# baryshnikova-lab/safepy

Measured on AMD Instinct MI355X. Metric: node-attribute enrichments/sec (nodes x attrs x perms), compute_pvalues permutation test, higher is better.
Workload: dtype u1 (bit-sliced integer counts; f64 outputs)

## Files before the change

### safepy_amd/csrc/attr.hip

```cpp
#include "common.h"

template <typename T>
__device__ __forceinline__ double load_attr(const void *raw, int64_t idx) {
    return static_cast<double>(reinterpret_cast<const T *>(raw)[idx]);
}

template <typename T, int GC>
__global__ __launch_bounds__(256) void k_attr_stats(const void *__restrict__ raw, int64_t n, int64_t m,
                                                    int64_t rs, int64_t cs, unsigned int *__restrict__ row_bits,
                                                    unsigned long long *__restrict__ acc ,
                                                    double *__restrict__ col_sum, unsigned long long *__restrict__ max_abs_bits,
                                                    unsigned int *__restrict__ col_nan, int64_t rows_per_block) {
    extern __shared__ unsigned int s_bits[];
    constexpr int RL = 256 / GC;
    const int cx = GC == 1 ? 0 : (threadIdx.x & (GC - 1));
    const int ry = GC == 1 ? threadIdx.x : (threadIdx.x / GC);
    const int lane = threadIdx.x & 63;
    const int64_t j = static_cast<int64_t>(blockIdx.x) * GC + cx;
    const int64_t n_words = (n + 31) / 32;
    __shared__ double s_sum[256];
    __shared__ double s_max[256];
    __shared__ unsigned int s_nan[256], s_other[256], s_nonint[256];
    const int64_t r_begin = static_cast<int64_t>(blockIdx.y) * rows_per_block;
    const int64_t r_end = r_begin + rows_per_block < n ? r_begin + rows_per_block : n;
// ... 111 lines not shown
            if (s_max[t] > tmx) tmx = s_max[t];
            t_nan += s_nan[t];
            t_other += s_other[t];
            t_nonint += s_nonint[t];
        }
        if (gridDim.y == 1) col_sum[j] = total;
        else atomicAdd(&col_sum[j], total);
        if (t_nan) atomicAdd(&col_nan[j], static_cast<unsigned int>(t_nan));
        if (t_other) atomicAdd(&acc[4 + (j & 63)], t_other);
        if (t_nonint) atomicAdd(&acc[68 + (j & 63)], t_nonint);
        const unsigned long long mine = static_cast<unsigned long long>(__double_as_longlong(tmx));
        if (mine > __builtin_nontemporal_load(max_abs_bits)) atomicMax(max_abs_bits, mine);
    }
}

__global__ __launch_bounds__(256) void k_stats_finish(unsigned long long *__restrict__ acc, const unsigned int *__restrict__ col_nan, int64_t m,
                                                      const unsigned int *__restrict__ bits, int64_t n, uint8_t *__restrict__ bytes,
                                                      unsigned long long *__restrict__ tail) {
    __shared__ unsigned int s_mx[4];
    __shared__ unsigned long long s_fold[2];
    unsigned int mx = 0;
    for (int64_t i = threadIdx.x; i < m; i += 256) mx = col_nan[i] > mx ? col_nan[i] : mx;
    for (int off = 32; off; off >>= 1) {
        const unsigned int o = __shfl_down(mx, off);
        mx = o > mx ? o : mx;
    }
    if ((threadIdx.x & 63) == 0) s_mx[threadIdx.x >> 6] = mx;
    if (threadIdx.x < 64) {
        unsigned long long a = acc[4 + threadIdx.x], b = acc[68 + threadIdx.x];
        for (int off = 32; off; off >>= 1) {
            a += __shfl_down(a, off);
            b += __shfl_down(b, off);
        }
        if (threadIdx.x == 0) s_fold[0] = a, s_fold[1] = b;
    }
    for (int64_t i = threadIdx.x; i < n; i += 256) bytes[i] = (bits[i >> 5] >> (i & 31)) & 1u;
    __syncthreads();
// ... 114 lines not shown
    SAFE_TRY(dev_alloc(&attr->sup_row, total));
    SAFE_HIP_CHECK(hipMemcpyAsync(attr->sup_ptr, attr->h_sup_ptr.data(), (m + 1) * sizeof(int32_t), hipMemcpyHostToDevice,
                                  ctx->stream));
    if (attr->dtype == SAFE_DTYPE_F32)
        hipLaunchKernelGGL(k_fill_support<float>, dim3(ceil_div(m * 64, 256)), dim3(256), 0, ctx->stream, attr->raw, n, m,
                           attr->row_stride, attr->col_stride, attr->sup_ptr, attr->sup_row);
    else
        hipLaunchKernelGGL(k_fill_support<double>, dim3(ceil_div(m * 64, 256)), dim3(256), 0, ctx->stream, attr->raw, n, m,
                           attr->row_stride, attr->col_stride, attr->sup_ptr, attr->sup_row);
    SAFE_HIP_CHECK(hipGetLastError());
    return SAFE_OK;
}

static size_t flags_block_bytes(int64_t n) { return static_cast<size_t>(ceil_div(n, 8)) * 8 + 32; }

int safe_attr_prepare(safe_attr *attr) {
    if (attr->stats_ready) return SAFE_OK;
    safe_ctx *ctx = attr->ctx;
    SAFE_HIP_CHECK(hipSetDevice(ctx->device));
    const int64_t n = attr->n, m = attr->m;
    const size_t flag_bytes = flags_block_bytes(n), tail_off = flag_bytes - 32;
    const int64_t n_words = (n + 31) / 32;
    SAFE_REQUIRE(n_words * sizeof(unsigned int) <= 150 * 1024, "safe_attr_stats: too many rows for the LDS row bitmap");
    void *tmp = nullptr;
    const size_t tmp_bytes = 132 * sizeof(unsigned long long) + static_cast<size_t>(n_words + m) * sizeof(unsigned int);
    SAFE_TRY(ctx_scratch(ctx, SCRATCH_ATTR_STATS, tmp_bytes, &tmp));
    unsigned long long *d_acc = static_cast<unsigned long long *>(tmp);
    unsigned int *d_rowbits = reinterpret_cast<unsigned int *>(d_acc + 132);
    unsigned int *d_colnan = d_rowbits + n_words;
    SAFE_HIP_CHECK(hipMemsetAsync(tmp, 0, tmp_bytes, ctx->stream));
    uint8_t *flags = nullptr;
    SAFE_TRY(ctx_block_alloc(ctx, flag_bytes, reinterpret_cast<void **>(&flags)));
    if (!attr->col_sum) SAFE_TRY(ctx_block_alloc(ctx, static_cast<size_t>(m) * sizeof(double), reinterpret_cast<void **>(&attr->col_sum)));
    const bool f32 = attr->dtype == SAFE_DTYPE_F32;
    const bool c_order = attr->col_stride == 1 && m > 1;
    if (c_order) SAFE_HIP_CHECK(hipMemsetAsync(attr->col_sum, 0, m * sizeof(double), ctx->stream));
#define STATS(T, GC, RPB)                                                                                          \
    do {                                                                                                           \
        if (n_words * sizeof(unsigned int) > 32 * 1024)                                                            \
            SAFE_HIP_CHECK(hipFuncSetAttribute(reinterpret_cast<const void *>(k_attr_stats<T, GC>),                \
                                               hipFuncAttributeMaxDynamicSharedMemorySize,                         \
                                               static_cast<int>(n_words * sizeof(unsigned int))));                 \
        hipLaunchKernelGGL((k_attr_stats<T, GC>), dim3(ceil_div(m, GC), ceil_div(n, RPB)), dim3(256),              \
                           n_words * sizeof(unsigned int), ctx->stream, attr->raw, n, m, attr->row_stride,         \
                           attr->col_stride, d_rowbits, d_acc, attr->col_sum, d_acc + 3, d_colnan,                 \
                           static_cast<int64_t>(RPB));                                                             \
    } while (0)
    if (c_order) {
        const int64_t groups = ceil_div(m, 64);
        const int64_t want_chunks = std::max<int64_t>(1, 2048 / groups);
        const int64_t rpb = std::max<int64_t>(256, ceil_div(ceil_div(n, want_chunks), 64) * 64);
        if (f32) STATS(float, 64, rpb);
        else STATS(double, 64, rpb);
    } else {
        if (f32) STATS(float, 1, n);
        else STATS(double, 1, n);
    }
#undef STATS
    hipLaunchKernelGGL(k_stats_finish, dim3(1), dim3(256), 0, ctx->stream, d_acc, d_colnan, m, d_rowbits, n, flags,
                       reinterpret_cast<unsigned long long *>(flags + tail_off));
    SAFE_HIP_CHECK(hipGetLastError());
    void *pinned = nullptr;
    SAFE_TRY(ctx_pinned(ctx, flag_bytes, &pinned));
    SAFE_HIP_CHECK(hipMemcpyAsync(pinned, flags, flag_bytes, hipMemcpyDeviceToHost, ctx->stream));
    SAFE_HIP_CHECK(safe_stream_sync(ctx->stream));
    const uint8_t *h_flags = static_cast<const uint8_t *>(pinned);
    unsigned long long h_acc[4];
    memcpy(h_acc, h_flags + tail_off, sizeof(h_acc));
    attr->n_other = static_cast<int64_t>(h_acc[0]);
    attr->max_nan_col = static_cast<int64_t>(h_acc[1]);
    attr->n_non_integer = static_cast<int64_t>(h_acc[2]);
    double mx;
    memcpy(&mx, &h_acc[3], sizeof(double));
    attr->max_abs = mx;
    if (!attr->flags_ready) {
        if (attr->row_flags) ctx_block_free(ctx, attr->row_flags, flag_bytes);
        attr->row_flags = flags;
        attr->flags_ready = true;
        int64_t cnt = 0;
        for (int64_t i = 0; i < n; ++i) cnt += h_flags[i] != 0;
        attr->n_rows_with_value = cnt;
        attr->h_row_flags.assign(h_flags, h_flags + n);
    } else {
// ... 387 lines not shown
    SAFE_REQUIRE(attr != nullptr, "safe_attr_nan_to_zero: attr is NULL");
    safe_ctx *ctx = attr->ctx;
    SAFE_HIP_CHECK(hipSetDevice(ctx->device));
    const int64_t count = attr->n * attr->m;
    const unsigned blocks = static_cast<unsigned>(std::min<int64_t>(ceil_div(count, 256), 8192));
    void *raw = const_cast<void *>(attr->raw);
    if (attr->dtype == SAFE_DTYPE_F32)
        hipLaunchKernelGGL(k_nan_to_zero<float>, dim3(blocks), dim3(256), 0, ctx->stream, reinterpret_cast<float *>(raw), count);
    else
        hipLaunchKernelGGL(k_nan_to_zero<double>, dim3(blocks), dim3(256), 0, ctx->stream, reinterpret_cast<double *>(raw), count);
    SAFE_HIP_CHECK(hipGetLastError());
    SAFE_HIP_CHECK(safe_stream_sync(ctx->stream));
    attr->stats_ready = false;
    attr->flags_ready = false;
    attr_free_support(attr);
    return SAFE_OK;
}

int safe_attr_download(safe_attr *attr, void *out_host) {
    SAFE_REQUIRE(attr && out_host, "safe_attr_download: NULL argument");
    safe_ctx *ctx = attr->ctx;
    SAFE_HIP_CHECK(hipSetDevice(ctx->device));
    const size_t bytes = static_cast<size_t>(attr->n) * attr->m * (attr->dtype == SAFE_DTYPE_F32 ? 4 : 8);
    SAFE_HIP_CHECK(hipMemcpyAsync(out_host, attr->raw, bytes, hipMemcpyDeviceToHost, ctx->stream));
    SAFE_HIP_CHECK(safe_stream_sync(ctx->stream));
    return SAFE_OK;
}

int safe_attr_destroy(safe_attr *attr) {
    if (!attr) return SAFE_OK;
    (void)hipSetDevice(attr->ctx->device);
    (void)safe_stream_sync(attr->ctx->stream);
    if (attr->owns_raw && attr->raw_pool_bytes) ctx_block_free(attr->ctx, const_cast<void *>(attr->raw), attr->raw_pool_bytes);
    else if (attr->owns_raw) (void)dev_free(attr->raw);
    ctx_block_free(attr->ctx, attr->row_flags, flags_block_bytes(attr->n));
    ctx_block_free(attr->ctx, attr->col_sum, static_cast<size_t>(attr->m) * sizeof(double));
    attr_free_support(attr);
    delete attr;
    return SAFE_OK;
}

int safe_attr_stats(safe_attr *attr, int64_t *n_other, int64_t *max_nan_col, int64_t *n_rows_with_value,
                    int64_t *n_non_integer) {
    SAFE_REQUIRE(attr != nullptr, "safe_attr_stats: attr is NULL");
    SAFE_TRY(safe_attr_prepare(attr));
    if (n_other) *n_other = attr->n_other;
    if (max_nan_col) *max_nan_col = attr->max_nan_col;
    if (n_rows_with_value) *n_rows_with_value = attr->n_rows_with_value;
    if (n_non_integer) *n_non_integer = attr->n_non_integer;
    return SAFE_OK;
}
// ... 24 lines not shown

int safe_attr_set_row_flags(safe_attr *attr, const uint8_t *flags_host) {
    SAFE_REQUIRE(attr && flags_host, "safe_attr_set_row_flags: NULL argument");
    safe_ctx *ctx = attr->ctx;
    SAFE_HIP_CHECK(hipSetDevice(ctx->device));
    const size_t flag_bytes = flags_block_bytes(attr->n);
    if (!attr->row_flags) SAFE_TRY(ctx_block_alloc(ctx, flag_bytes, reinterpret_cast<void **>(&attr->row_flags)));
    std::vector<uint8_t> tmp(flag_bytes, 0);
    int64_t cnt = 0;
    for (int64_t i = 0; i < attr->n; ++i) {
        tmp[i] = flags_host[i] ? 1 : 0;
        cnt += tmp[i];
    }
    SAFE_HIP_CHECK(hipMemcpyAsync(attr->row_flags, tmp.data(), flag_bytes, hipMemcpyHostToDevice, ctx->stream));
    SAFE_HIP_CHECK(safe_stream_sync(ctx->stream));
    attr->flags_ready = true;
    attr->n_rows_with_value = cnt;
    attr->h_row_flags.assign(tmp.begin(), tmp.begin() + attr->n);
    return SAFE_OK;
}

}
```

### safepy_amd/csrc/common.h

```cpp
#pragma once
#include <hip/hip_runtime.h>

#include <algorithm>
#include <cstdarg>
#include <cmath>
#include <cstdint>
#include <cstdio>
#include <cstdlib>
#include <cstring>
#include <condition_variable>
#include <memory>
#include <mutex>
#include <atomic>
#include <string>
#include <thread>
#include <vector>

#include "safe_hip.h"
#include "bits_plan.h"

#define SAFE_WAVE 64
#define SAFE_PAD_U16 0xFFFFu

void safe_set_error(const char *fmt, ...);
// ... 274 lines not shown
    int32_t *row_ptr = nullptr;
    int32_t *col = nullptr;
    int64_t n_slices = 0;
    int32_t *sell_row = nullptr;
    int32_t *sell_pos = nullptr;
    int64_t *slice_off = nullptr;
    int32_t *slice_width = nullptr;
    int32_t *sell_col = nullptr;
    int64_t sell_entries = 0;
    uint16_t *sell_col2 = nullptr;
    uint16_t *sell_col2b = nullptr;
    std::vector<int32_t> h_slice_width;
    BitsTaskPlan bits_plan;
    void *bits_plan_pinned = nullptr;
    size_t bits_plan_pinned_bytes = 0;
    std::vector<int64_t> h_slice_off;
    std::vector<int32_t> h_row_count;
    double *dist = nullptr;
    int32_t *at_ptr = nullptr;
    int32_t *at_col = nullptr;
    std::vector<double> h_xy;
    bool blocks_ready = false;
    int64_t bs_groups = 0;
    int64_t bs_blocks = 0;
    int64_t bs_pieces = 0;
    int64_t bs_src = 0;
    int32_t *bs_order = nullptr;
    int32_t *bs_rowmap = nullptr;
    int32_t *bs_rowcnt = nullptr;
    int32_t *bs_grpmax = nullptr;
// ... 63 lines not shown
    const void *raw = nullptr;
    bool owns_raw = false;
    size_t raw_pool_bytes = 0;
    uint8_t *row_flags = nullptr;
    std::vector<uint8_t> h_row_flags;
    bool flags_ready = false;
    bool stats_ready = false;
    int64_t n_other = 0, max_nan_col = 0, n_rows_with_value = 0, n_non_integer = 0;
    double *col_sum = nullptr;
    double max_abs = 0.0;
    int32_t *sup_ptr = nullptr;
    int32_t *sup_row = nullptr;
    int64_t n_ones = 0;
    std::vector<int32_t> h_sup_ptr;
    size_t sup_ptr_pool_bytes = 0, sup_row_pool_bytes = 0;
};

struct DrawStream;

struct safe_perms {
    safe_ctx *ctx = nullptr;
    int64_t n = 0;
    int64_t count = 0;
    int64_t k = 0;
    std::vector<int32_t> h_movable;
    DrawStream *stream = nullptr;
    int64_t generated = 0, enqueued = 0;
    std::vector<int64_t> stages;
    std::vector<hipEvent_t> chunk_done;
    std::vector<uint32_t> h_local;
    std::thread drawer;
// ... 98 lines not shown
```

### safepy_amd/csrc/ctx.hip

```cpp
#include "common.h"
#include "ring.h"

#include <atomic>
#include <chrono>
#include <map>
#include <thread>

static thread_local char g_error[1024] = "";

void safe_trace(const char *what) {
    static const bool on = getenv("SAFE_HIP_TRACE") != nullptr;
    if (!on) return;
    static const auto t0 = std::chrono::steady_clock::now();
    fprintf(stderr, "[safe_hip %9.3f ms] %s\n",
            std::chrono::duration<double, std::milli>(std::chrono::steady_clock::now() - t0).count(), what);
}

void safe_warn_diagnostic(const char *name) {
    static std::mutex mu;
    static std::vector<std::string> seen;
    std::lock_guard<std::mutex> lk(mu);
    for (const std::string &n : seen)
        if (n == name) return;
    seen.emplace_back(name);
    fprintf(stderr, "[safe_hip] WARNING: diagnostic switch %s is set: kernels skip work, the results of this process are INVALID\n", name);
}

void safe_set_error(const char *fmt, ...) {
    va_list ap;
    va_start(ap, fmt);
    vsnprintf(g_error, sizeof(g_error), fmt, ap);
    va_end(ap);
}

static std::atomic<int> g_blocking_sync{-1};
std::atomic<long long> g_alloc_calls{0}, g_live_blocks{0};

static bool blocking_sync_on() {
    int v = g_blocking_sync.load(std::memory_order_relaxed);
    if (v < 0) {
// ... 455 lines not shown
```

### safepy_amd/csrc/enrich.hip

```cpp
#include <algorithm>
#include <cmath>
#include <numeric>

#include "common.h"
#include "hyp_math.h"

template <typename T, int BN, int PLANES>
__global__ __launch_bounds__(256) void k_tile_prep(const void *__restrict__ raw, int64_t n, int64_t rs, int64_t cs,
                                                   int64_t col0, int64_t mloc, int64_t n_tiles,
                                                   double *__restrict__ bt) {
    const int64_t idx = static_cast<int64_t>(blockIdx.x) * 256 + threadIdx.x;
    const int64_t total = n_tiles * (n + 1) * BN;
    if (idx >= total) return;
    const int c = static_cast<int>(idx % BN);
    const int64_t row = (idx / BN) % (n + 1);
    const int64_t tile = idx / (static_cast<int64_t>(BN) * (n + 1));
    const int64_t j = tile * BN + c;
    double v = 0.0, v2 = 0.0, nn = 0.0;
    if (row < n && j < mloc) {
        const T x = reinterpret_cast<const T *>(raw)[row * rs + (col0 + j) * cs];
        if (x == x) {
            v = static_cast<double>(x);
            v2 = static_cast<double>(static_cast<T>(x * x));
            nn = 1.0;
// ... 1159 lines not shown
    blk_sum<LV, 2, 1>(ids, lane, nblk, o0, o1);
#pragma unroll
    for (int l = 0; l < BT_LV; ++l) {
        oo0[l] = l < LV ? o0[l < LV ? l : 0] : 0u;
        oo1[l] = l < LV ? o1[l < LV ? l : 0] : 0u;
        obs[l * 64 + lane] = oo0[l];
        obs[(BT_LV + l) * 64 + lane] = oo1[l];
    }
}

__global__ __launch_bounds__(256) void k_bits_observed(int64_t n, const int32_t *__restrict__ sell_row,
                                                       const int64_t *__restrict__ slice_off,
                                                       const int32_t *__restrict__ slice_width,
                                                       const uint16_t *__restrict__ sell_col2b, int64_t n_slices,
                                                       const uint2 *__restrict__ bbits, int64_t mloc,
                                                       uint32_t *__restrict__ obs, double *__restrict__ ns_out) {
    extern __shared__ unsigned int lds[];
    uint2 *T = reinterpret_cast<uint2 *>(lds);
    if ((uint32_t)(uintptr_t)((__attribute__((address_space(3))) unsigned int *)lds) != 0u) __builtin_trap();
    const int wave = __builtin_amdgcn_readfirstlane(threadIdx.x >> 6), lane = threadIdx.x & 63;
    const int64_t wg = blockIdx.x, s = static_cast<int64_t>(blockIdx.y) * 4 + wave;
    load_word_column(T, bbits + wg * (n + 1), n);
    __syncthreads();
    if (s >= n_slices) return;
    const int wdt = __builtin_amdgcn_readfirstlane(slice_width[s]);
    const u32x4 *ids = reinterpret_cast<const u32x4 *>(sell_col2b) + slice_off[s] / 8;
    uint32_t *my_obs = obs + (wg * n_slices + s) * (2 * BT_LV * 64);
    uint32_t oo0[BT_LV], oo1[BT_LV];
    if (wdt <= 8) observed_wave<4>(ids, lane, wdt >> 3, my_obs, oo0, oo1);
    else if (wdt <= 56) observed_wave<6>(ids, lane, wdt >> 3, my_obs, oo0, oo1);
    else if (wdt <= 248) observed_wave<8>(ids, lane, wdt >> 3, my_obs, oo0, oo1);
    else if (wdt <= 504) observed_wave<9>(ids, lane, wdt >> 3, my_obs, oo0, oo1);
    else observed_wave<BT_LV>(ids, lane, wdt >> 3, my_obs, oo0, oo1);
    if (ns_out) {
        const int32_t row = sell_row[s * 64 + lane];
        uint16_t *tile = reinterpret_cast<uint16_t *>(lds + 2 * ((n + 2) & ~int64_t(1)) + 4) + wave * (64 * 66);
// ... 343 lines not shown
    const int64_t n = attr->n;
    const bool f32 = attr->dtype == SAFE_DTYPE_F32;
    if (attr->col_stride == 1 && attr->row_stride != 1) {
        const dim3 grid(n_wg, ceil_div(n + 1, 4)), block(256);
        if (f32) hipLaunchKernelGGL(k_bits_prep_rowmajor<float>, grid, block, 0, ctx->stream, attr->raw, n, attr->row_stride,
                                    attr->col_stride, col0, mloc, n_wg, d_bits);
        else hipLaunchKernelGGL(k_bits_prep_rowmajor<double>, grid, block, 0, ctx->stream, attr->raw, n, attr->row_stride,
                                attr->col_stride, col0, mloc, n_wg, d_bits);
    } else {
        const dim3 grid(ceil_div(n_wg * (n + 1), 256)), block(256);
        if (f32) hipLaunchKernelGGL(k_bits_prep<float>, grid, block, 0, ctx->stream, attr->raw, n, attr->row_stride,
                                    attr->col_stride, col0, mloc, n_wg, d_bits);
        else hipLaunchKernelGGL(k_bits_prep<double>, grid, block, 0, ctx->stream, attr->raw, n, attr->row_stride,
                                attr->col_stride, col0, mloc, n_wg, d_bits);
    }
}


template <bool TABLE>
__global__ __launch_bounds__(64) void k_counts_bits(const int32_t *__restrict__ sell_row,
                                                    const int64_t *__restrict__ slice_off,
                                                    const int32_t *__restrict__ slice_width,
                                                    const int32_t *__restrict__ sell_col, int64_t n,
                                                    const uint2 *__restrict__ bbits, int64_t mloc,
                                                    double *__restrict__ out, HypLookup hl) {
    const int64_t s = blockIdx.x, wg = blockIdx.y;
    const int lane = threadIdx.x;
    const int32_t row = sell_row[s * 64 + lane];
    const int32_t *cols = sell_col + slice_off[s] + lane;
    const int wdt = slice_width[s];
// ... 582 lines not shown
                        tail.n_major, tail.n_chunks, tail.wpc);
    const std::vector<int4> &recs = bits_plan_records(plan, form);
    const size_t bytes = recs.size() * sizeof(int4);
    if (nbr->bits_plan_pinned_bytes < bytes) {
        SAFE_HIP_CHECK(safe_stream_sync(ctx->stream));
        if (nbr->bits_plan_pinned) SAFE_HIP_CHECK(hipHostFree(nbr->bits_plan_pinned));
        nbr->bits_plan_pinned = nullptr;
        nbr->bits_plan_pinned_bytes = 0;
        g_alloc_calls.fetch_add(1, std::memory_order_relaxed);
        SAFE_HIP_CHECK(hipHostMalloc(&nbr->bits_plan_pinned, bytes + 4096, hipHostMallocDefault));
        nbr->bits_plan_pinned_bytes = bytes + 4096;
    } else {
        SAFE_HIP_CHECK(safe_stream_sync(ctx->stream));
    }
    memcpy(nbr->bits_plan_pinned, recs.data(), bytes);
    plan.key = plan_key;
    return SAFE_OK;
}

constexpr int BITS_NS = 2;

struct BitsBuffers {
    uint2 *d_bits = nullptr;
    int4 *d_tasks = nullptr;
    unsigned int *d_queue = nullptr, *d_gl = nullptr;
    int64_t n_pad = 0, entries_pad = 0;
    uint16_t *d_ids[BITS_NS] = {nullptr, nullptr};
    uint16_t *d_ids_tail = nullptr;
    uint32_t *d_obs = nullptr;
};
static int bits_call_buffers(safe_ctx *ctx, const safe_nbr *nbr, const BitsForm &form, const BitsTail &tail, int64_t mloc, int64_t span,
                             int64_t tail_span, BitsBuffers *b) {
    const size_t n_task = bits_plan_records(nbr->bits_plan, form).size();
    const int64_t n_launch = tail.n_major + tail.n_chunks;
    void *ws = nullptr;
    SAFE_TRY(ctx_scratch(ctx, SCRATCH_TASKS, n_task * sizeof(int4) + (8 * n_launch + 4) * sizeof(unsigned int), &ws));
    b->d_tasks = static_cast<int4 *>(ws);
    b->d_queue = reinterpret_cast<unsigned int *>(b->d_tasks + n_task);
    b->n_pad = nbr->n_slices * 64;
    SAFE_TRY(ctx_scratch(ctx, SCRATCH_COUNTERS, static_cast<size_t>(b->n_pad) * mloc * sizeof(unsigned int), reinterpret_cast<void **>(&b->d_gl)));
    SAFE_HIP_CHECK(hipMemcpyAsync(b->d_tasks, nbr->bits_plan_pinned, n_task * sizeof(int4), hipMemcpyHostToDevice, ctx->stream));
    SAFE_HIP_CHECK(hipMemsetAsync(b->d_queue, 0, 8 * n_launch * sizeof(unsigned int), ctx->stream));
    SAFE_HIP_CHECK(hipMemsetAsync(b->d_gl, 0, static_cast<size_t>(b->n_pad) * mloc * sizeof(unsigned int), ctx->stream));
    safe_trace("launch_bits: buffers ready");
    b->entries_pad = (nbr->sell_entries + 1024 + 255) / 256 * 256;
    for (int s = 0; s < BITS_NS; ++s)
        SAFE_TRY(ctx_scratch(ctx, scratch_pair(SCRATCH_STREAM_A, s), static_cast<size_t>(span) * b->entries_pad * sizeof(uint16_t), reinterpret_cast<void **>(&b->d_ids[s])));
    if (tail.n_chunks)
        SAFE_TRY(ctx_scratch(ctx, SCRATCH_BITS_TAIL_IDS, static_cast<size_t>(tail_span) * b->entries_pad * sizeof(uint16_t), reinterpret_cast<void **>(&b->d_ids_tail)));
    return SAFE_OK;
}

static int bits_observe(safe_ctx *ctx, const safe_nbr *nbr, const BitsForm &form, int64_t mloc, double *ns_out, BitsBuffers *b) {
    const int64_t n_wg = ceil_div(mloc, 64);
    SAFE_TRY(ctx_scratch(ctx, SCRATCH_BITS_OBSERVED, static_cast<size_t>(n_wg) * nbr->n_slices * 2 * BT_LV * 64 * sizeof(uint32_t),
                         reinterpret_cast<void **>(&b->d_obs)));
    const size_t lds_obs = form.lds_bytes + (ns_out ? 4 * 64 * 66 * sizeof(uint16_t) : 0);
    SAFE_HIP_CHECK(hipFuncSetAttribute(reinterpret_cast<const void *>(k_bits_observed), hipFuncAttributeMaxDynamicSharedMemorySize,
                                       static_cast<int>(lds_obs)));
    hipLaunchKernelGGL(k_bits_observed, dim3(n_wg, ceil_div(nbr->n_slices, 4)), dim3(256), lds_obs, ctx->stream, nbr->n, nbr->sell_row,
                       nbr->slice_off, nbr->slice_width, nbr->sell_col2b, nbr->n_slices, b->d_bits, mloc, b->d_obs, ns_out);
    SAFE_HIP_CHECK(hipGetLastError());
    return SAFE_OK;
}

static int bits_tail_lists(safe_ctx *ctx, const safe_nbr *nbr, safe_perms *perms, const std::vector<int64_t> &starts, const BitsTail &tail,
                           const BitsBuffers &b, hipEvent_t *plain) {
    hipStream_t tail_ps = ctx->more_streams[1], kstreams[BITS_NS] = {ctx->stream, ctx->side_stream};
    const int64_t n_stage = static_cast<int64_t>(starts.size()) - 1, entries_pad = b.entries_pad;
    SAFE_HIP_CHECK(hipStreamWaitEvent(tail_ps, plain[0], 0));
    for (int64_t t = tail.n_major; t < n_stage; ++t) {
        SAFE_TRY(perms_wait(perms, starts[t + 1], tail_ps));
        hipLaunchKernelGGL(k_permute_cols, dim3(ceil_div(entries_pad, 4096), starts[t + 1] - starts[t]), dim3(256),
                           static_cast<size_t>(perms->stride16) * sizeof(uint16_t), tail_ps, perms->table16, perms->stride16,
                           nbr->sell_col2b, nbr->sell_entries, entries_pad, starts[t], starts[t + 1] - starts[t],
                           static_cast<uint32_t>(8 * nbr->n), b.d_ids_tail + (starts[t] - tail.p_split) * entries_pad, 3);
// ... 53 lines not shown
                            (void *)&n_pad};
        void *pre_args[] = {(void *)&n, (void *)&ids_c, (void *)&entries_pad, (void *)&nbr->sell_row, (void *)&nbr->slice_off,
                            (void *)&nbr->slice_width, (void *)&nbr->sell_col2, (void *)&nbr->n_slices, (void *)&b.d_bits, (void *)&n_tasks,
                            (void *)&d_tasks, (void *)&p_base, (void *)&p_limit, (void *)&queue_c, (void *)&mloc, (void *)&b.d_gl,
                            (void *)&n_pad, (void *)&ns_out};
        SAFE_HIP_CHECK(hipLaunchKernel(kfn, dim3(grid), dim3(form.block), blk ? blk_args : pre_args, form.lds_bytes, ks));
        if (in_tail) chunk_final(c, ks);
        SAFE_HIP_CHECK(hipGetLastError());
        SAFE_HIP_CHECK(hipEventRecord(fr.ev[2 * c + 1], ks));
    }
    return SAFE_OK;
}

static int launch_bits(safe_ctx *ctx, safe_nbr *nbr, safe_attr *attr, safe_perms *perms, int64_t col0, int64_t col1,
                       const PermOut &out) {
    const int64_t n = nbr->n, mloc = col1 - col0, n_wg = ceil_div(mloc, 64), P = perms->count;
    const BitsForm form = bits_form(n, nbr->max_count, nbr->sell_col2 != nullptr, 160 * 1024);
    SAFE_REQUIRE(form.kind != BITS_NONE, "launch_bits: no bit-sliced form for %lld nodes with neighborhoods of up to %lld members",
                 static_cast<long long>(n), static_cast<long long>(nbr->max_count));
    safe_trace("launch_bits: enter");
    BitsBuffers b;
    SAFE_TRY(ctx_scratch(ctx, SCRATCH_OPERANDS, static_cast<size_t>(n_wg) * (n + 1) * sizeof(uint2), reinterpret_cast<void **>(&b.d_bits)));
    launch_bits_prep(ctx, attr, col0, mloc, n_wg, b.d_bits);
    safe_trace("launch_bits: prep launched");
    const BitsSwitches sw = bits_switches(ctx);
    int64_t span = 1;
    const std::vector<int64_t> starts = perm_launch_starts(perms, &span, 1, sw.tail_frac > 0.0);
    ctx->xc_made = 0;
    const BitsTail tail = bits_tail_split(ctx->xc_want, ctx->xc_cols, safe_ctx::XC_MAX, form.kind == BITS_BLK, starts, P, mloc, sw.tail_frac);
    const int64_t n_tail = tail.n_chunks, tail_span = P - tail.p_split;
    const int64_t n_launch = tail.n_major + n_tail;
    const int per_cu = static_cast<int>(std::max<size_t>(1, std::min<size_t>(8, (160 * 1024) / bits_lds_bytes(n, perms->stride16))));
    SAFE_TRY(bits_task_plan(ctx, nbr, form, tail, starts, static_cast<int64_t>(ctx->num_cu) * per_cu, mloc));
    safe_trace("launch_bits: tasks built");
    SAFE_TRY(bits_call_buffers(ctx, nbr, form, tail, mloc, span, tail_span, &b));
    const void *kfn = bits_form_kernel(form, sw.dbg);
    if (!kfn) return SAFE_E_INVALID;
    SAFE_HIP_CHECK(hipFuncSetAttribute(kfn, hipFuncAttributeMaxDynamicSharedMemorySize, static_cast<int>(form.lds_bytes)));
// ... 18 lines not shown
        safe_trace("launch_bits: column chunks enqueued");
        if (ctx->xc_callback) ctx->xc_callback(ctx->xc_user);
    }
    SAFE_TRY(span_frame_join(ctx, fr));
    SAFE_TRY(enrich_finalize_counts(ctx, b.d_gl, b.n_pad, nbr->sell_row, mloc, P, out, nullptr));
    SAFE_HIP_CHECK(hipGetLastError());
    safe_trace("launch_bits: all enqueued");
    SAFE_TRY(span_frame_close(ctx, fr));
    safe_trace("launch_bits: synced");
    if (sw.dbg & 128) blk_trace_dump(static_cast<int>(n_launch));
    return SAFE_OK;
}

static int launch_counts_bits(safe_ctx *ctx, safe_nbr *nbr, safe_attr *attr, int64_t col0, int64_t col1, double *out_dev) {
    const int64_t n = nbr->n, mloc = col1 - col0, n_wg = ceil_div(mloc, 64);
    uint2 *d_bits = nullptr;
    SAFE_TRY(ctx_scratch(ctx, SCRATCH_OPERANDS, static_cast<size_t>(n_wg) * (n + 1) * sizeof(uint2), reinterpret_cast<void **>(&d_bits)));
    launch_bits_prep(ctx, attr, col0, mloc, n_wg, d_bits);
    SAFE_HIP_CHECK(hipEventRecord(ctx->k0, ctx->stream));
    hipLaunchKernelGGL(k_counts_bits<false>, dim3(nbr->n_slices, n_wg), dim3(64), 0, ctx->stream, nbr->sell_row, nbr->slice_off,
                       nbr->slice_width, nbr->sell_col, n, d_bits, mloc, out_dev, HypLookup{});
    SAFE_HIP_CHECK(hipGetLastError());
    SAFE_HIP_CHECK(hipEventRecord(ctx->k1, ctx->stream));
    ctx->last_kernel.name = "k_counts_bits";
    return SAFE_OK;
}

static size_t ldsf64_bytes(int64_t n, int64_t stride16) {
    return (8 * static_cast<size_t>(n + 1) + static_cast<size_t>(stride16) + 4) * sizeof(unsigned int);
}

static int launch_lds_f64(safe_ctx *ctx, safe_nbr *nbr, safe_attr *attr, safe_perms *perms, int64_t col0, int64_t col1,
                          bool z, const PermOut &out_in) {
// ... 136 lines not shown
    hl.nes = nes_dev;
    hl.nes_binary = nb_dev;
    hl.enriched = d_enr;
    if (split) {
        int rc = mfma_counts_split_emit(ctx, nbr, split, hl);
        if (rc == SAFE_OK && enriched_f64) {
            hipLaunchKernelGGL(k_u32_to_f64, dim3(ceil_div(mloc, 256)), dim3(256), 0, ctx->stream, d_enr, enriched_f64, mloc);
            if (hipGetLastError() != hipSuccess) rc = SAFE_E_HIP;
        }
        (void)safe_stream_sync(hs);
        (void)hipEventDestroy(ids_done);
        SAFE_TRY(rc);
    } else if (use_mfma) {
        SAFE_TRY(launch_mfma_counts(ctx, nbr, attr, col0, col1, hl));
    } else {
        uint2 *d_bits = nullptr;
        SAFE_TRY(ctx_scratch(ctx, SCRATCH_OPERANDS, static_cast<size_t>(n_wg) * (n + 1) * sizeof(uint2), reinterpret_cast<void **>(&d_bits)));
        launch_bits_prep(ctx, attr, col0, mloc, n_wg, d_bits);
        SAFE_HIP_CHECK(hipEventRecord(ctx->k0, ctx->stream));
        hipLaunchKernelGGL(k_counts_bits<true>, dim3(nbr->n_slices, n_wg), dim3(64), 0, ctx->stream, nbr->sell_row, nbr->slice_off,
                           nbr->slice_width, nbr->sell_col, n, d_bits, mloc, static_cast<double *>(nullptr), hl);
        SAFE_HIP_CHECK(hipGetLastError());
        SAFE_HIP_CHECK(hipEventRecord(ctx->k1, ctx->stream));
        ctx->last_kernel.name = "k_counts_bits<hypergeom>";
    }
    if (split && enriched_f64 && enriched_done) *enriched_done = true;
    SAFE_HIP_CHECK(safe_stream_sync(ctx->stream));
    *fused = true;
    return SAFE_OK;
}

__global__ __launch_bounds__(256) void k_counts_to_outputs(const double *__restrict__ counts_neg, const double *__restrict__ counts_pos,
                                                           const double *__restrict__ ns, int64_t total, int64_t m, int64_t n_perm,
// ... 553 lines not shown
```

### safepy_amd/csrc/nbr.hip

```cpp
#include <algorithm>
#include <cmath>
#include <numeric>

#include "common.h"

static double squared_threshold(double nr) {
    if (!(nr > 0.0)) return 0.0;
    if (std::isinf(nr)) return nr;
    double c = nr * nr;
    if (std::isinf(c)) return c;
    while (c > 0.0 && std::sqrt(c) >= nr) c = std::nextafter(c, 0.0);
    while (std::sqrt(c) < nr) c = std::nextafter(c, INFINITY);
    return c;
}

__global__ __launch_bounds__(256) void k_euclid_bits(const double *__restrict__ xy, int64_t n, double thr_sq,
                                                     uint64_t *__restrict__ bits, int64_t words) {
    __shared__ double sx[64], sy[64];
    const int64_t w = blockIdx.x;
    const int64_t i = static_cast<int64_t>(blockIdx.y) * 256 + threadIdx.x;
    const int64_t j0 = w * 64;
    if (threadIdx.x < 64) {
        const int64_t j = j0 + threadIdx.x;
        sx[threadIdx.x] = j < n ? xy[2 * j] : 0.0;
// ... 600 lines not shown
    }
    SAFE_REQUIRE(src.n >= 2 || n_ranks == 0, "%s: rank %lld is outside [0, 0): one node has no pair", who, (long long)ranks[0]);
    *keys = pre;
    return SAFE_OK;
}

static void nbr_free(safe_nbr *nbr) {
    if (!nbr) return;
    for (const void *q : {(const void *)nbr->bits, (const void *)nbr->row_ptr, (const void *)nbr->col, (const void *)nbr->sell_row,
                          (const void *)nbr->sell_pos, (const void *)nbr->slice_off, (const void *)nbr->slice_width,
                          (const void *)nbr->sell_col, (const void *)nbr->sell_col2, (const void *)nbr->sell_col2b,
                          (const void *)nbr->dist, (const void *)nbr->at_ptr, (const void *)nbr->at_col})
        (void)dev_free(q);
    nbr_free_blocks(nbr);
    if (nbr->bits_plan_pinned) (void)hipHostFree(nbr->bits_plan_pinned);
    delete nbr;
}

using NbrPtr = std::unique_ptr<safe_nbr, void (*)(safe_nbr *)>;

static int nbr_new(safe_ctx *ctx, int64_t n, NbrPtr *out) {
    SAFE_REQUIRE(n >= 1 && n < (1ll << 31) - 64, "neighborhood size n=%lld out of range", (long long)n);
    NbrPtr nbr(new safe_nbr(), nbr_free);
    nbr->ctx = ctx;
    nbr->n = n;
    nbr->words = ceil_div(n, 64);
    SAFE_TRY(dev_alloc(&nbr->bits, static_cast<size_t>(n) * nbr->words));
    *out = std::move(nbr);
    return SAFE_OK;
}
// ... 550 lines not shown
```

Measured before the change: 6892 billion.

## Build attribute bit planes during stats sweep and fold buffer clears into observe kernel

Adds a binary-attribute sweep kernel that computes column statistics and packs the 64-column bit planes in one pass over the raw matrix. Later bit-sliced count launches reuse these cached planes instead of rerunning the bits-prep kernel per call. The task plan is kept resident on the device, and the counter and queue zeroing moves into the observed-counts kernel, removing per-call H2D copies and memsets. If the attribute is not strictly binary, the sweep falls back to the old stats pass, costing an extra pass and some memory for the planes.

After: 6988 billion (median of 6 runs). 1.01x the previous value.

```diff
diff --git a/safepy_amd/csrc/attr.hip b/safepy_amd/csrc/attr.hip
--- a/safepy_amd/csrc/attr.hip
+++ b/safepy_amd/csrc/attr.hip
@@ -1,4 +1,5 @@
 #include "common.h"
+#include "attr_plan.h"
 
 template <typename T>
 __device__ __forceinline__ double load_attr(const void *raw, int64_t idx) {
@@ -149,13 +150,92 @@
     }
 }
 
+template <typename T>
+__global__ __launch_bounds__(256) void k_attr_sweep(const T *__restrict__ raw, int64_t n, int64_t m, int64_t cs, int64_t rows_per_block,
+                                                    unsigned int *__restrict__ row_bits, unsigned long long *__restrict__ acc,
+                                                    unsigned int *__restrict__ col_nan, unsigned int *__restrict__ col_one,
+                                                    uint2 *__restrict__ bbits) {
+    __shared__ unsigned int s_nan[4][64], s_one[4][64], s_other[4];
+    const int wave = threadIdx.x >> 6, lane = threadIdx.x & 63;
+    const int64_t wg = blockIdx.x, j0 = wg * 64;
+    const int n_cols = static_cast<int>(m - j0 < 64 ? m - j0 : 64);
+    const int64_t r_begin = static_cast<int64_t>(blockIdx.y) * rows_per_block;
+    const int64_t r_end = r_begin + rows_per_block < n ? r_begin + rows_per_block : n;
+    const T *base = raw + j0 * cs;
+    uint2 *planes = bbits + wg * (n + 1);
+    unsigned int c_nan = 0, c_one = 0, c_other = 0;
+    for (int64_t r0 = r_begin + wave * 64; r0 < r_end; r0 += 256) {
+        const int64_t r = r0 + lane;
+        const bool inb = r < n;
+        const T *p = base + (inb ? r : r0);
+        uint32_t w0 = 0, w1 = 0;
+        bool has = false;
+        auto take = [&](int a, T v) {
+            const bool nan = v != v, one = v == static_cast<T>(1), zero = v == static_cast<T>(0);
+            const bool is_nan = inb && nan, is_one = inb && one;
+            const unsigned int k_nan = __popcll(__ballot(is_nan)), k_one = __popcll(__ballot(is_one));
+            c_nan += lane == a ? k_nan : 0u;
+            c_one += lane == a ? k_one : 0u;
+            c_other += (inb && !nan && !one && !zero) ? 1u : 0u;
+            has = has || (inb && !nan);
+            if (a < 32) w0 |= (is_one ? 1u : 0u) << (a & 31);
+            else w1 |= (is_one ? 1u : 0u) << (a & 31);
+        };
+        if (n_cols == 64) {
+#pragma unroll
+            for (int a0 = 0; a0 < 64; a0 += 16) {
+                T x[16];
+#pragma unroll
+                for (int u = 0; u < 16; ++u) x[u] = p[(a0 + u) * cs];
+#pragma unroll
+                for (int u = 0; u < 16; ++u) take(a0 + u, x[u]);
+            }
+        } else {
+            for (int a = 0; a < n_cols; ++a) take(a, p[a * cs]);
+        }
+        if (inb) planes[r] = make_uint2(w0, w1);
+        const unsigned long long bal = __ballot(has);
+        if (lane == 0 && bal) {
+            const unsigned int lo = static_cast<unsigned int>(bal), hi = static_cast<unsigned int>(bal >> 32);
+            if (lo & ~row_bits[r0 >> 5]) atomicOr(&row_bits[r0 >> 5], lo);
+            if (hi && (hi & ~row_bits[(r0 >> 5) + 1])) atomicOr(&row_bits[(r0 >> 5) + 1], hi);
+        }
+    }
+    for (int off = 32; off; off >>= 1) c_other += __shfl_down(c_other, off);
+    s_nan[wave][lane] = c_nan;
+    s_one[wave][lane] = c_one;
+    if (lane == 0) s_other[wave] = c_other;
+    __syncthreads();
+    if (threadIdx.x < 64) {
+        const unsigned int t_nan = s_nan[0][lane] + s_nan[1][lane] + s_nan[2][lane] + s_nan[3][lane];
+        const unsigned int t_one = s_one[0][lane] + s_one[1][lane] + s_one[2][lane] + s_one[3][lane];
+        if (lane < n_cols) {
+            if (t_nan) atomicAdd(&col_nan[j0 + lane], t_nan);
+            if (t_one) atomicAdd(&col_one[j0 + lane], t_one);
+        }
+        const bool any_one = __ballot(lane < n_cols && t_one != 0) != 0ull;
+        if (lane == 0) {
+            const unsigned long long t_other = static_cast<unsigned long long>(s_other[0]) + s_other[1] + s_other[2] + s_other[3];
+            if (t_other) atomicAdd(&acc[4 + (wg & 63)], t_other);
+            const unsigned long long one_bits = static_cast<unsigned long long>(__double_as_longlong(1.0));
+            if (any_one && one_bits > __builtin_nontemporal_load(&acc[3])) atomicMax(&acc[3], one_bits);
+            if (blockIdx.y == 0) planes[n] = make_uint2(0u, 0u);
+        }
+    }
+}
+
 __global__ __launch_bounds__(256) void k_stats_finish(unsigned long long *__restrict__ acc, const unsigned int *__restrict__ col_nan, int64_t m,
                                                       const unsigned int *__restrict__ bits, int64_t n, uint8_t *__restrict__ bytes,
-                                                      unsigned long long *__restrict__ tail) {
+                                                      unsigned long long *__restrict__ tail, const unsigned int *__restrict__ col_one,
+                                                      double *__restrict__ col_sum) {
     __shared__ unsigned int s_mx[4];
     __shared__ unsigned long long s_fold[2];
     unsigned int mx = 0;
-    for (int64_t i = threadIdx.x; i < m; i += 256) mx = col_nan[i] > mx ? col_nan[i] : mx;
+    for (int64_t i = threadIdx.x; i < m; i += 256) {
+        const unsigned int c = col_nan[i];
+        if (col_one) col_sum[i] = static_cast<double>(col_one[i]);
+        mx = c > mx ? c : mx;
+    }
     for (int off = 32; off; off >>= 1) {
         const unsigned int o = __shfl_down(mx, off);
         mx = o > mx ? o : mx;
@@ -300,25 +380,47 @@
 
 static size_t flags_block_bytes(int64_t n) { return static_cast<size_t>(ceil_div(n, 8)) * 8 + 32; }
 
-int safe_attr_prepare(safe_attr *attr) {
-    if (attr->stats_ready) return SAFE_OK;
+void attr_drop_planes(safe_attr *attr) {
+    ctx_block_free(attr->ctx, attr->planes, attr->planes_bytes);
+    attr->planes = nullptr;
+    attr->planes_bytes = 0;
+}
+
+const uint2 *attr_bit_planes(const safe_attr *attr, int64_t col0, int64_t col1) {
+    if (!attr->planes || !binary_head_on() || !planes_serve_block(col0, col1, attr->m)) return nullptr;
+    return attr->planes + (col0 / 64) * (attr->n + 1);
+}
+
+static int stats_pass(safe_attr *attr, bool sweep, uint8_t *flags, void *pinned) {
     safe_ctx *ctx = attr->ctx;
-    SAFE_HIP_CHECK(hipSetDevice(ctx->device));
     const int64_t n = attr->n, m = attr->m;
     const size_t flag_bytes = flags_block_bytes(n), tail_off = flag_bytes - 32;
     const int64_t n_words = (n + 31) / 32;
-    SAFE_REQUIRE(n_words * sizeof(unsigned int) <= 150 * 1024, "safe_attr_stats: too many rows for the LDS row bitmap");
     void *tmp = nullptr;
-    const size_t tmp_bytes = 132 * sizeof(unsigned long long) + static_cast<size_t>(n_words + m) * sizeof(unsigned int);
+    const size_t tmp_bytes = 132 * sizeof(unsigned long long) + static_cast<size_t>(n_words + 2 * m) * sizeof(unsigned int);
     SAFE_TRY(ctx_scratch(ctx, SCRATCH_ATTR_STATS, tmp_bytes, &tmp));
     unsigned long long *d_acc = static_cast<unsigned long long *>(tmp);
     unsigned int *d_rowbits = reinterpret_cast<unsigned int *>(d_acc + 132);
-    unsigned int *d_colnan = d_rowbits + n_words;
+    unsigned int *d_colnan = d_rowbits + n_words, *d_colone = d_colnan + m;
     SAFE_HIP_CHECK(hipMemsetAsync(tmp, 0, tmp_bytes, ctx->stream));
-    uint8_t *flags = nullptr;
-    SAFE_TRY(ctx_block_alloc(ctx, flag_bytes, reinterpret_cast<void **>(&flags)));
-    if (!attr->col_sum) SAFE_TRY(ctx_block_alloc(ctx, static_cast<size_t>(m) * sizeof(double), reinterpret_cast<void **>(&attr->col_sum)));
     const bool f32 = attr->dtype == SAFE_DTYPE_F32;
+    if (sweep) {
+        const int64_t n_wg = ceil_div(m, 64), rpb = sweep_rows_per_block(n, n_wg);
+        const dim3 grid(static_cast<unsigned int>(n_wg), static_cast<unsigned int>(ceil_div(n, rpb)));
+        if (f32)
+            hipLaunchKernelGGL(k_attr_sweep<float>, grid, dim3(256), 0, ctx->stream, static_cast<const float *>(attr->raw), n, m,
+                               attr->col_stride, rpb, d_rowbits, d_acc, d_colnan, d_colone, attr->planes);
+        else
+            hipLaunchKernelGGL(k_attr_sweep<double>, grid, dim3(256), 0, ctx->stream, static_cast<const double *>(attr->raw), n, m,
+                               attr->col_stride, rpb, d_rowbits, d_acc, d_colnan, d_colone, attr->planes);
+        hipLaunchKernelGGL(k_stats_finish, dim3(1), dim3(256), 0, ctx->stream, d_acc, d_colnan, m, d_rowbits, n, flags,
+                           reinterpret_cast<unsigned long long *>(flags + tail_off), d_colone, attr->col_sum);
+        SAFE_HIP_CHECK(hipGetLastError());
+        SAFE_HIP_CHECK(hipMemcpyAsync(pinned, flags, flag_bytes, hipMemcpyDeviceToHost, ctx->stream));
+        SAFE_HIP_CHECK(safe_stream_sync(ctx->stream));
+        return SAFE_OK;
+    }
+    SAFE_REQUIRE(n_words * sizeof(unsigned int) <= 150 * 1024, "safe_attr_stats: too many rows for the LDS row bitmap");
     const bool c_order = attr->col_stride == 1 && m > 1;
     if (c_order) SAFE_HIP_CHECK(hipMemsetAsync(attr->col_sum, 0, m * sizeof(double), ctx->stream));
 #define STATS(T, GC, RPB)                                                                                          \
@@ -344,15 +446,41 @@
     }
 #undef STATS
     hipLaunchKernelGGL(k_stats_finish, dim3(1), dim3(256), 0, ctx->stream, d_acc, d_colnan, m, d_rowbits, n, flags,
-                       reinterpret_cast<unsigned long long *>(flags + tail_off));
+                       reinterpret_cast<unsigned long long *>(flags + tail_off), static_cast<const unsigned int *>(nullptr),
+                       static_cast<double *>(nullptr));
     SAFE_HIP_CHECK(hipGetLastError());
+    SAFE_HIP_CHECK(hipMemcpyAsync(pinned, flags, flag_bytes, hipMemcpyDeviceToHost, ctx->stream));
+    SAFE_HIP_CHECK(safe_stream_sync(ctx->stream));
+    return SAFE_OK;
+}
+
+int safe_attr_prepare(safe_attr *attr) {
+    if (attr->stats_ready) return SAFE_OK;
+    safe_ctx *ctx = attr->ctx;
+    SAFE_HIP_CHECK(hipSetDevice(ctx->device));
+    const int64_t n = attr->n, m = attr->m;
+    const size_t flag_bytes = flags_block_bytes(n), tail_off = flag_bytes - 32;
+    SAFE_REQUIRE(static_cast<size_t>((n + 31) / 32) * sizeof(unsigned int) <= 150 * 1024, "safe_attr_stats: too many rows for the LDS row bitmap");
+    uint8_t *flags = nullptr;
+    SAFE_TRY(ctx_block_alloc(ctx, flag_bytes, reinterpret_cast<void **>(&flags)));
+    if (!attr->col_sum) SAFE_TRY(ctx_block_alloc(ctx, static_cast<size_t>(m) * sizeof(double), reinterpret_cast<void **>(&attr->col_sum)));
     void *pinned = nullptr;
     SAFE_TRY(ctx_pinned(ctx, flag_bytes, &pinned));
-    SAFE_HIP_CHECK(hipMemcpyAsync(pinned, flags, flag_bytes, hipMemcpyDeviceToHost, ctx->stream));
-    SAFE_HIP_CHECK(safe_stream_sync(ctx->stream));
     const uint8_t *h_flags = static_cast<const uint8_t *>(pinned);
     unsigned long long h_acc[4];
+    bool sweep = binary_head_on() && attr->row_stride == 1 && (attr->col_stride == n || m == 1);
+    if (sweep && !attr->planes) {
+        const size_t bytes = static_cast<size_t>(ceil_div(m, 64)) * (n + 1) * sizeof(uint2);
+        SAFE_TRY(ctx_block_alloc(ctx, bytes, reinterpret_cast<void **>(&attr->planes)));
+        attr->planes_bytes = bytes;
+    }
+    SAFE_TRY(stats_pass(attr, sweep, flags, pinned));
     memcpy(h_acc, h_flags + tail_off, sizeof(h_acc));
+    if (sweep && h_acc[0] != 0) {
+        attr_drop_planes(attr);
+        SAFE_TRY(stats_pass(attr, false, flags, pinned));
+        memcpy(h_acc, h_flags + tail_off, sizeof(h_acc));
+    }
     attr->n_other = static_cast<int64_t>(h_acc[0]);
     attr->max_nan_col = static_cast<int64_t>(h_acc[1]);
     attr->n_non_integer = static_cast<int64_t>(h_acc[2]);
@@ -770,6 +898,7 @@
     attr->stats_ready = false;
     attr->flags_ready = false;
     attr_free_support(attr);
+    attr_drop_planes(attr);
     return SAFE_OK;
 }
 
@@ -791,6 +920,7 @@
     else if (attr->owns_raw) (void)dev_free(attr->raw);
     ctx_block_free(attr->ctx, attr->row_flags, flags_block_bytes(attr->n));
     ctx_block_free(attr->ctx, attr->col_sum, static_cast<size_t>(attr->m) * sizeof(double));
+    attr_drop_planes(attr);
     attr_free_support(attr);
     delete attr;
     return SAFE_OK;
@@ -845,6 +975,7 @@
     }
     SAFE_HIP_CHECK(hipMemcpyAsync(attr->row_flags, tmp.data(), flag_bytes, hipMemcpyHostToDevice, ctx->stream));
     SAFE_HIP_CHECK(safe_stream_sync(ctx->stream));
+    attr_drop_planes(attr);
     attr->flags_ready = true;
     attr->n_rows_with_value = cnt;
     attr->h_row_flags.assign(tmp.begin(), tmp.begin() + attr->n);
diff --git a/safepy_amd/csrc/attr_plan.h b/safepy_amd/csrc/attr_plan.h
--- /dev/null
+++ b/safepy_amd/csrc/attr_plan.h
@@ -0,0 +1,14 @@
+#pragma once
+#include <cstdint>
+
+static inline int64_t sweep_rows_per_block(int64_t n, int64_t n_wg) {
+    const int64_t chunks = n_wg >= 1024 ? 1 : 1024 / (n_wg < 1 ? 1 : n_wg);
+    const int64_t rows = (n + chunks - 1) / chunks;
+    const int64_t rounded = (rows + 128) / 256 * 256;
+    return rounded < 256 ? 256 : rounded;
+}
+
+static inline bool planes_serve_block(int64_t col0, int64_t col1, int64_t m) {
+    if (col0 < 0 || col1 <= col0 || col1 > m) return false;
+    return col0 % 64 == 0 && (col1 == m || col1 % 64 == 0);
+}
diff --git a/safepy_amd/csrc/common.h b/safepy_amd/csrc/common.h
--- a/safepy_amd/csrc/common.h
+++ b/safepy_amd/csrc/common.h
@@ -312,6 +312,8 @@
     BitsTaskPlan bits_plan;
     void *bits_plan_pinned = nullptr;
     size_t bits_plan_pinned_bytes = 0;
+    int4 *bits_plan_dev = nullptr;
+    size_t bits_plan_dev_bytes = 0;
     std::vector<int64_t> h_slice_off;
     std::vector<int32_t> h_row_count;
     double *dist = nullptr;
@@ -405,7 +407,12 @@
     int64_t n_ones = 0;
     std::vector<int32_t> h_sup_ptr;
     size_t sup_ptr_pool_bytes = 0, sup_row_pool_bytes = 0;
-};
+    uint2 *planes = nullptr;
+    size_t planes_bytes = 0;
+};
+const uint2 *attr_bit_planes(const safe_attr *attr, int64_t col0, int64_t col1);
+void attr_drop_planes(safe_attr *attr);
+bool binary_head_on();
 
 struct DrawStream;
 
diff --git a/safepy_amd/csrc/ctx.hip b/safepy_amd/csrc/ctx.hip
--- a/safepy_amd/csrc/ctx.hip
+++ b/safepy_amd/csrc/ctx.hip
@@ -24,6 +24,11 @@
         if (n == name) return;
     seen.emplace_back(name);
     fprintf(stderr, "[safe_hip] WARNING: diagnostic switch %s is set: kernels skip work, the results of this process are INVALID\n", name);
+}
+
+bool binary_head_on() {
+    const char *e = getenv("SAFE_HIP_BINARY_HEAD");
+    return !(e && !strcmp(e, "0"));
 }
 
 void safe_set_error(const char *fmt, ...) {
diff --git a/safepy_amd/csrc/enrich.hip b/safepy_amd/csrc/enrich.hip
--- a/safepy_amd/csrc/enrich.hip
+++ b/safepy_amd/csrc/enrich.hip
@@ -1197,12 +1197,21 @@
                                                        const int32_t *__restrict__ slice_width,
                                                        const uint16_t *__restrict__ sell_col2b, int64_t n_slices,
                                                        const uint2 *__restrict__ bbits, int64_t mloc,
-                                                       uint32_t *__restrict__ obs, double *__restrict__ ns_out) {
+                                                       uint32_t *__restrict__ obs, double *__restrict__ ns_out,
+                                                       unsigned int *__restrict__ gl_counts, int64_t n_pad,
+                                                       unsigned int *__restrict__ queue, int n_queue) {
     extern __shared__ unsigned int lds[];
     uint2 *T = reinterpret_cast<uint2 *>(lds);
     if ((uint32_t)(uintptr_t)((__attribute__((address_space(3))) unsigned int *)lds) != 0u) __builtin_trap();
     const int wave = __builtin_amdgcn_readfirstlane(threadIdx.x >> 6), lane = threadIdx.x & 63;
     const int64_t wg = blockIdx.x, s = static_cast<int64_t>(blockIdx.y) * 4 + wave;
+    if (gl_counts && s < n_slices) {
+        const int n_valid = static_cast<int>(mloc - wg * 64 < 64 ? mloc - wg * 64 : 64);
+        unsigned int *z = gl_counts + wg * 64 * n_pad + s * 64 + 4 * (lane & 15);
+        for (int a = lane >> 4; a < n_valid; a += 4) *reinterpret_cast<uint4 *>(z + static_cast<int64_t>(a) * n_pad) = make_uint4(0u, 0u, 0u, 0u);
+    }
+    if (queue && blockIdx.x == 0 && blockIdx.y == 0)
+        for (int i = threadIdx.x; i < n_queue; i += 256) queue[i] = 0u;
     load_word_column(T, bbits + wg * (n + 1), n);
     __syncthreads();
     if (s >= n_slices) return;
@@ -1576,6 +1585,19 @@
         else hipLaunchKernelGGL(k_bits_prep<double>, grid, block, 0, ctx->stream, attr->raw, n, attr->row_stride,
                                 attr->col_stride, col0, mloc, n_wg, d_bits);
     }
+}
+
+static int bits_operand(safe_ctx *ctx, const safe_attr *attr, int64_t col0, int64_t col1, const uint2 **out) {
+    if (const uint2 *planes = attr_bit_planes(attr, col0, col1)) {
+        *out = planes;
+        return SAFE_OK;
+    }
+    const int64_t mloc = col1 - col0, n_wg = ceil_div(mloc, 64);
+    uint2 *d_bits = nullptr;
+    SAFE_TRY(ctx_scratch(ctx, SCRATCH_OPERANDS, static_cast<size_t>(n_wg) * (attr->n + 1) * sizeof(uint2), reinterpret_cast<void **>(&d_bits)));
+    launch_bits_prep(ctx, attr, col0, mloc, n_wg, d_bits);
+    *out = d_bits;
+    return SAFE_OK;
 }
 
 
@@ -2188,6 +2210,15 @@
         SAFE_HIP_CHECK(safe_stream_sync(ctx->stream));
     }
     memcpy(nbr->bits_plan_pinned, recs.data(), bytes);
+    if (nbr->bits_plan_dev_bytes < bytes) {
+        SAFE_HIP_CHECK(dev_free(nbr->bits_plan_dev));
+        nbr->bits_plan_dev = nullptr;
+        nbr->bits_plan_dev_bytes = 0;
+        SAFE_TRY(dev_alloc_bytes(reinterpret_cast<void **>(&nbr->bits_plan_dev), bytes + 4096));
+        nbr->bits_plan_dev_bytes = bytes + 4096;
+    }
+    SAFE_HIP_CHECK(hipMemcpyAsync(nbr->bits_plan_dev, nbr->bits_plan_pinned, bytes, hipMemcpyHostToDevice, ctx->stream));
+    SAFE_HIP_CHECK(safe_stream_sync(ctx->stream));
     plan.key = plan_key;
     return SAFE_OK;
 }
@@ -2195,13 +2226,15 @@
 constexpr int BITS_NS = 2;
 
 struct BitsBuffers {
-    uint2 *d_bits = nullptr;
+    const uint2 *d_bits = nullptr;
     int4 *d_tasks = nullptr;
     unsigned int *d_queue = nullptr, *d_gl = nullptr;
     int64_t n_pad = 0, entries_pad = 0;
     uint16_t *d_ids[BITS_NS] = {nullptr, nullptr};
     uint16_t *d_ids_tail = nullptr;
     uint32_t *d_obs = nullptr;
+    bool cleared_by_observe = false;
+    int n_queue = 0;
 };
 static int bits_call_buffers(safe_ctx *ctx, const safe_nbr *nbr, const BitsForm &form, const BitsTail &tail, int64_t mloc, int64_t span,
                              int64_t tail_span, BitsBuffers *b) {
@@ -2213,9 +2246,15 @@
     b->d_queue = reinterpret_cast<unsigned int *>(b->d_tasks + n_task);
     b->n_pad = nbr->n_slices * 64;
     SAFE_TRY(ctx_scratch(ctx, SCRATCH_COUNTERS, static_cast<size_t>(b->n_pad) * mloc * sizeof(unsigned int), reinterpret_cast<void **>(&b->d_gl)));
-    SAFE_HIP_CHECK(hipMemcpyAsync(b->d_tasks, nbr->bits_plan_pinned, n_task * sizeof(int4), hipMemcpyHostToDevice, ctx->stream));
-    SAFE_HIP_CHECK(hipMemsetAsync(b->d_queue, 0, 8 * n_launch * sizeof(unsigned int), ctx->stream));
-    SAFE_HIP_CHECK(hipMemsetAsync(b->d_gl, 0, static_cast<size_t>(b->n_pad) * mloc * sizeof(unsigned int), ctx->stream));
+    const bool head = binary_head_on();
+    b->cleared_by_observe = head && form.kind == BITS_BLK;
+    if (head) b->d_tasks = nbr->bits_plan_dev;
+    else SAFE_HIP_CHECK(hipMemcpyAsync(b->d_tasks, nbr->bits_plan_pinned, n_task * sizeof(int4), hipMemcpyHostToDevice, ctx->stream));
+    if (!b->cleared_by_observe) {
+        SAFE_HIP_CHECK(hipMemsetAsync(b->d_queue, 0, 8 * n_launch * sizeof(unsigned int), ctx->stream));
+        SAFE_HIP_CHECK(hipMemsetAsync(b->d_gl, 0, static_cast<size_t>(b->n_pad) * mloc * sizeof(unsigned int), ctx->stream));
+    }
+    b->n_queue = static_cast<int>(8 * n_launch);
     safe_trace("launch_bits: buffers ready");
     b->entries_pad = (nbr->sell_entries + 1024 + 255) / 256 * 256;
     for (int s = 0; s < BITS_NS; ++s)
@@ -2233,7 +2272,9 @@
     SAFE_HIP_CHECK(hipFuncSetAttribute(reinterpret_cast<const void *>(k_bits_observed), hipFuncAttributeMaxDynamicSharedMemorySize,
                                        static_cast<int>(lds_obs)));
     hipLaunchKernelGGL(k_bits_observed, dim3(n_wg, ceil_div(nbr->n_slices, 4)), dim3(256), lds_obs, ctx->stream, nbr->n, nbr->sell_row,
-                       nbr->slice_off, nbr->slice_width, nbr->sell_col2b, nbr->n_slices, b->d_bits, mloc, b->d_obs, ns_out);
+                       nbr->slice_off, nbr->slice_width, nbr->sell_col2b, nbr->n_slices, b->d_bits, mloc, b->d_obs, ns_out,
+                       b->cleared_by_observe ? b->d_gl : static_cast<unsigned int *>(nullptr), b->n_pad,
+                       b->cleared_by_observe ? b->d_queue : static_cast<unsigned int *>(nullptr), b->n_queue);
     SAFE_HIP_CHECK(hipGetLastError());
     return SAFE_OK;
 }
@@ -2317,14 +2358,13 @@
 
 static int launch_bits(safe_ctx *ctx, safe_nbr *nbr, safe_attr *attr, safe_perms *perms, int64_t col0, int64_t col1,
                        const PermOut &out) {
-    const int64_t n = nbr->n, mloc = col1 - col0, n_wg = ceil_div(mloc, 64), P = perms->count;
+    const int64_t n = nbr->n, mloc = col1 - col0, P = perms->count;
     const BitsForm form = bits_form(n, nbr->max_count, nbr->sell_col2 != nullptr, 160 * 1024);
     SAFE_REQUIRE(form.kind != BITS_NONE, "launch_bits: no bit-sliced form for %lld nodes with neighborhoods of up to %lld members",
                  static_cast<long long>(n), static_cast<long long>(nbr->max_count));
     safe_trace("launch_bits: enter");
     BitsBuffers b;
-    SAFE_TRY(ctx_scratch(ctx, SCRATCH_OPERANDS, static_cast<size_t>(n_wg) * (n + 1) * sizeof(uint2), reinterpret_cast<void **>(&b.d_bits)));
-    launch_bits_prep(ctx, attr, col0, mloc, n_wg, b.d_bits);
+    SAFE_TRY(bits_operand(ctx, attr, col0, col1, &b.d_bits));
     safe_trace("launch_bits: prep launched");
     const BitsSwitches sw = bits_switches(ctx);
     int64_t span = 1;
@@ -2373,9 +2413,8 @@
 
 static int launch_counts_bits(safe_ctx *ctx, safe_nbr *nbr, safe_attr *attr, int64_t col0, int64_t col1, double *out_dev) {
     const int64_t n = nbr->n, mloc = col1 - col0, n_wg = ceil_div(mloc, 64);
-    uint2 *d_bits = nullptr;
-    SAFE_TRY(ctx_scratch(ctx, SCRATCH_OPERANDS, static_cast<size_t>(n_wg) * (n + 1) * sizeof(uint2), reinterpret_cast<void **>(&d_bits)));
-    launch_bits_prep(ctx, attr, col0, mloc, n_wg, d_bits);
+    const uint2 *d_bits = nullptr;
+    SAFE_TRY(bits_operand(ctx, attr, col0, col1, &d_bits));
     SAFE_HIP_CHECK(hipEventRecord(ctx->k0, ctx->stream));
     hipLaunchKernelGGL(k_counts_bits<false>, dim3(nbr->n_slices, n_wg), dim3(64), 0, ctx->stream, nbr->sell_row, nbr->slice_off,
                        nbr->slice_width, nbr->sell_col, n, d_bits, mloc, out_dev, HypLookup{});
@@ -2542,9 +2581,8 @@
     } else if (use_mfma) {
         SAFE_TRY(launch_mfma_counts(ctx, nbr, attr, col0, col1, hl));
     } else {
-        uint2 *d_bits = nullptr;
-        SAFE_TRY(ctx_scratch(ctx, SCRATCH_OPERANDS, static_cast<size_t>(n_wg) * (n + 1) * sizeof(uint2), reinterpret_cast<void **>(&d_bits)));
-        launch_bits_prep(ctx, attr, col0, mloc, n_wg, d_bits);
+        const uint2 *d_bits = nullptr;
+        SAFE_TRY(bits_operand(ctx, attr, col0, col1, &d_bits));
         SAFE_HIP_CHECK(hipEventRecord(ctx->k0, ctx->stream));
         hipLaunchKernelGGL(k_counts_bits<true>, dim3(nbr->n_slices, n_wg), dim3(64), 0, ctx->stream, nbr->sell_row, nbr->slice_off,
                            nbr->slice_width, nbr->sell_col, n, d_bits, mloc, static_cast<double *>(nullptr), hl);
diff --git a/safepy_amd/csrc/nbr.hip b/safepy_amd/csrc/nbr.hip
--- a/safepy_amd/csrc/nbr.hip
+++ b/safepy_amd/csrc/nbr.hip
@@ -638,6 +638,7 @@
         (void)dev_free(q);
     nbr_free_blocks(nbr);
     if (nbr->bits_plan_pinned) (void)hipHostFree(nbr->bits_plan_pinned);
+    (void)dev_free(nbr->bits_plan_dev);
     delete nbr;
 }
 
```
